# Abhipray/audio-codec

Hardware: AMD Instinct MI355X
Metric: audio channel-frames/s encode (48 kHz, 1024-line long blocks, 128 kb/s/ch) (higher is better)
Workload: dtype f64

## Files before the change

### audio-codec_amd/_lib.py

```python
import ctypes
import os

HERE = os.path.dirname(os.path.abspath(__file__))
LIB_PATH = os.environ.get("PACX_LIB") or os.path.join(HERE, "libpacx.so")

PACX_ABI_VERSION = 7
PCM_I16, PCM_F64 = 0, 1
FLAG_LAST, FLAG_CUR, FLAG_NEXT = 1, 2, 4
ST_SHORT, ST_ZERO_SUBBLOCK, ST_ALLOC_CAP, ST_VQ_UNDEFINED, ST_GUARD, ST_MALFORMED = 1, 2, 4, 8, 16, 32
ST_REF_RAISES = 64
ST_RATE_CAP = 128
RATE_STEP = 32
RATE_TARGET_GRID = 64
BAND_CAND = 16
E_ARG, E_UNSUPPORTED = -1, -2
REF_SCALAR_SBR_ERROR = "'numpy.int64' object does not support item assignment"
MAX_BANDS = 32
SUB = 8

c_double_p = ctypes.POINTER(ctypes.c_double)
c_int32_p = ctypes.POINTER(ctypes.c_int32)


class PacxSmrTables(ctypes.Structure):
# ... 58 lines not shown
class PacxPcm(ctypes.Structure):
    _fields_ = [
        ("data", ctypes.c_void_p),
        ("dtype", ctypes.c_int32),
        ("n_channels", ctypes.c_int32),
        ("n_frames", ctypes.c_int64),
        ("frame_stride", ctypes.c_int64),
        ("channel_stride", ctypes.c_int64),
        ("sample_stride", ctypes.c_int64),
    ]


_P = ctypes.c_void_p
SIGNATURES = {
    "pacx_abi_version": (ctypes.c_int, []),
    "pacx_create": (ctypes.c_int, [ctypes.POINTER(PacxConfig), ctypes.POINTER(_P)]),
    "pacx_destroy": (None, [_P]),
    "pacx_last_error": (ctypes.c_char_p, [_P]),
    "pacx_band_stride": (ctypes.c_int, [_P]),
    "pacx_payload_stride": (ctypes.c_int, [_P]),
    "pacx_reserve": (ctypes.c_int, [_P, ctypes.c_int64]),
    "pacx_tables_exact": (ctypes.c_int, [_P]),
    "pacx_default_bands": (ctypes.c_int, [ctypes.c_int, ctypes.c_int, c_int32_p, c_int32_p]),
    "pacx_mdct_batch": (ctypes.c_int, [_P, ctypes.POINTER(PacxPcm), _P, ctypes.c_int, _P, _P, _P]),
    "pacx_smr_batch": (ctypes.c_int, [_P, ctypes.POINTER(PacxPcm), _P, ctypes.c_int, _P, _P, _P, _P]),
    "pacx_bitalloc_batch": (ctypes.c_int, [_P, ctypes.c_int64, ctypes.c_int, _P, ctypes.c_int, _P, _P, _P, _P]),
    "pacx_quantize_batch": (ctypes.c_int, [_P, ctypes.c_int64, _P, _P, _P, ctypes.c_int, _P, _P, _P]),
    "pacx_encode_batch": (ctypes.c_int, [_P, ctypes.POINTER(PacxPcm), _P, _P, _P, _P, _P, _P, _P]),
    "pacx_encode_pack_batch": (ctypes.c_int, [_P, ctypes.POINTER(PacxPcm), _P, _P, _P, _P, _P, _P, _P, _P, _P]),
    "pacx_encode_vq_batch": (ctypes.c_int, [_P, ctypes.POINTER(PacxPcm), _P, _P, _P, _P, _P, _P, _P, _P,
                                            ctypes.c_int32, _P]),
    "pacx_pack_batch": (ctypes.c_int, [_P, ctypes.c_int64, ctypes.c_int, _P, _P, _P, _P, _P, _P, _P, _P, _P]),
    "pacx_gather_body": (ctypes.c_int, [_P, ctypes.c_int64, _P, _P, _P, ctypes.c_int64, _P, _P]),
    "pacx_window_batch": (ctypes.c_int, [_P, ctypes.c_int, ctypes.c_int64, _P, _P, _P]),
    "pacx_window_table_batch": (ctypes.c_int, [_P, _P, ctypes.c_int, ctypes.c_int64, _P, _P, _P]),
    "pacx_quantize_uniform": (ctypes.c_int, [_P, ctypes.c_int64, _P, ctypes.c_int, _P, _P]),
    "pacx_scale_factor": (ctypes.c_int, [_P, ctypes.c_int64, _P, ctypes.c_int, ctypes.c_int, _P, _P]),
    "pacx_mantissa": (ctypes.c_int, [_P, ctypes.c_int64, _P, ctypes.c_int, ctypes.c_int, ctypes.c_int, _P, _P]),
    "pacx_dequantize_uniform": (ctypes.c_int, [_P, ctypes.c_int64, _P, ctypes.c_int, _P, _P]),
    "pacx_dequantize": (ctypes.c_int, [_P, ctypes.c_int64, _P, ctypes.c_int, ctypes.c_int, ctypes.c_int, _P, _P]),
    "pacx_mantissa_fp": (ctypes.c_int, [_P, ctypes.c_int64, _P, ctypes.c_int, ctypes.c_int, ctypes.c_int, _P, _P]),
    "pacx_dequantize_fp": (ctypes.c_int, [_P, ctypes.c_int64, _P, ctypes.c_int, ctypes.c_int, ctypes.c_int, _P, _P]),
    "pacx_imdct_batch": (ctypes.c_int, [_P, ctypes.c_int64, ctypes.c_int, _P, _P, _P]),
    "pacx_mdct_direct_batch": (ctypes.c_int, [_P, ctypes.c_int64, ctypes.c_int, ctypes.c_int, ctypes.c_int, _P, _P, _P]),
    "pacx_transient_detect_f64": (ctypes.c_int, [_P, ctypes.c_int64, ctypes.c_int, ctypes.c_int, _P, ctypes.c_double, _P, _P]),
    "pacx_unpack_batch": (ctypes.c_int, [_P, ctypes.c_int64, _P, ctypes.c_int, _P, _P, _P, _P, _P, _P, _P, _P, _P]),
    "pacx_set_side_fork": (ctypes.c_int, [_P, ctypes.c_int]),
    "pacx_smr_generic_batch": (ctypes.c_int, [_P, ctypes.c_int64, ctypes.c_int, _P, _P, ctypes.POINTER(PacxSmrTables), _P, _P,
                                              _P, _P]),
    "pacx_decode_batch": (ctypes.c_int, [_P, ctypes.c_int64, ctypes.c_int, _P, _P, _P, _P, _P, _P, _P, _P]),
    "pacx_decode_sbr_batch": (ctypes.c_int, [_P, ctypes.c_int64, ctypes.c_int, _P, _P, _P, _P, _P, ctypes.c_int, _P, _P,
                                             _P, _P, _P]),
    "pacx_decode_vq_batch": (ctypes.c_int, [_P, ctypes.c_int64, ctypes.c_int, _P, ctypes.c_int, _P, _P, _P, _P, _P,
                                            _P, _P, _P, _P, _P]),
    "pacx_transient_flags": (ctypes.c_int, [_P, ctypes.POINTER(PacxPcm), _P, _P, _P]),
    "pacx_bitalloc_generic": (ctypes.c_int, [_P, ctypes.c_int64, ctypes.c_int, _P, _P, ctypes.c_int, _P, _P, _P]),
    "pacx_index_body": (ctypes.c_int, [_P, _P, ctypes.c_int64, ctypes.c_int, ctypes.c_int, ctypes.c_int64, _P, _P, _P, _P]),
    "pacx_overlap_add_pcm": (ctypes.c_int, [_P, ctypes.c_int64, ctypes.c_int, _P, _P, ctypes.c_int, _P, _P]),
    "pacx_nmr_batch": (ctypes.c_int, [_P, ctypes.POINTER(PacxPcm), _P, _P, _P, _P, _P, _P, _P, _P]),
    "pacx_nmr_summary": (ctypes.c_int, [_P, ctypes.c_int64, ctypes.c_int, _P, _P, _P, _P]),
    "pacx_encode_pack_nmr_batch": (ctypes.c_int, [_P, ctypes.POINTER(PacxPcm), _P, ctypes.c_double, ctypes.c_double,
                                                  _P, _P, _P, _P, _P, _P, _P, _P, _P]),
    "pacx_encode_pack_budget_batch": (ctypes.c_int, [_P, ctypes.POINTER(PacxPcm), _P, _P, _P, _P, _P, _P, _P, _P, _P,
                                                     _P]),
    "pacx_rate_curve_layout": (ctypes.c_int, [_P, ctypes.c_double, c_int32_p, c_int32_p]),
    "pacx_rate_curve_batch": (ctypes.c_int, [_P, ctypes.POINTER(PacxPcm), _P, ctypes.c_double, ctypes.c_int32, _P, _P, _P,
# ... 73 lines not shown
```

### audio-codec_amd/csrc/k_misc.hip

```cpp
#include "pacx_launch.h"

__global__ void k_window(const double *__restrict__ win, long long n_rows, int len,
                         const double *__restrict__ x, double *__restrict__ y)
{
    const long long i = (long long)blockIdx.x * blockDim.x + threadIdx.x;
    if (i < n_rows * len)
        y[i] = win[i % len] * x[i];
}

__global__ void k_quant_elem(int op, long long n, const double *__restrict__ x, int scale, int a, int b,
                             int64_t *__restrict__ out)
{
    const long long i = (long long)blockIdx.x * blockDim.x + threadIdx.x;
    if (i >= n)
        return;
    const double v = x[i];
    if (op == 0) {
        const int64_t mag = pacx_quant_mag(fabs(v), a);
        out[i] = (v < 0.0 ? ((int64_t)1 << (a - 1)) : 0) + mag;
    } else if (op == 1) {
        out[i] = pacx_scale_factor(fabs(v), a, b);
    } else if (op == 2) {
        out[i] = pacx_mantissa(v, scale, a, b);
    } else {
// ... 299 lines not shown
    if (lane == 63) {
        ws[wv] = ss;
        wl[wv] = sl;
    }
    __syncthreads();
    int at_s = ss - ns, at_l = sl - nl, all_s = 0, all_l = 0;
#pragma unroll
    for (int w = 0; w < NW; ++w) {
        at_s += w < wv ? ws[w] : 0;
        at_l += w < wv ? wl[w] : 0;
        all_s += ws[w];
        all_l += wl[w];
    }
    for (int j = 0; j < per; ++j) {
        if (!((valid >> j) & 1ull))
            break;
        const long long f = f0 + j;
        if ((shorts >> j) & 1ull) {
            for (int c = 0; c < n_ch; ++c)
                list_short[at_s * n_ch + c] = (int32_t)(f * n_ch + c);
            ++at_s;
        } else {
            for (int c = 0; c < n_ch; ++c)
                list_long[at_l * n_ch + c] = (int32_t)(f * n_ch + c);
            ++at_l;
        }
    }
    if (tid == 0) {
        counts[0] = all_l * n_ch;
        counts[1] = all_s * n_ch;
    }
}

void pacx_k::pacx_launch_frame_lists(const uint8_t *flags, long long n_frames, int n_ch, int32_t *list_long,
                             int32_t *list_short, int32_t *counts, hipStream_t st)
{
    if (n_frames <= 0)
        return;
    if (n_frames <= LISTS_SMALL_MAX) {
        hipLaunchKernelGGL(k_frame_lists_small, dim3(1), dim3(LISTS_SMALL_THREADS), 0, st, flags, n_frames, n_ch, list_long,
                           list_short, counts);
        return;
    }
    (void)hipMemsetAsync(counts, 0, 2 * sizeof(int32_t), st);
    hipLaunchKernelGGL(k_frame_lists, dim3((unsigned)((n_frames + 255) / 256)), dim3(256), 0, st, flags, n_frames,
                       n_ch, list_long, list_short, counts);
}

void pacx_k::pacx_launch_transient_f64(long long n_blocks, int n_ch, int n, const double *blocks, double thresh, uint8_t *out,
                               hipStream_t st)
{
    if (n_blocks > 0)
        hipLaunchKernelGGL(k_transient_f64, dim3((unsigned)n_blocks), dim3(64), 0, st, n_blocks, n_ch, n, blocks, thresh,
                           out);
}

void pacx_k::pacx_launch_transient(const PacxPcmView &in, long long n_hops, int hop, uint8_t *transient,
                           uint8_t *flags, hipStream_t st)
{
    if (n_hops > 0)
        hipLaunchKernelGGL(k_transient, dim3((unsigned)n_hops), dim3(64), 0, st, in, n_hops, hop, transient);
    if (flags)
        hipLaunchKernelGGL(k_stream_flags, dim3((unsigned)((n_hops + 2 + 255) / 256)), dim3(256), 0, st,
                           transient, n_hops, flags);
}

// ... 40 lines not shown
```

### audio-codec_amd/csrc/k_quant.hip

```cpp
#include "pacx_launch.h"
#include "wave_fft.h"
#include "quant_dev.h"

__global__ __launch_bounds__(64) void k_bitalloc(PacxTables T, const uint8_t *__restrict__ flags, int n_ch,
                                                long long n_cf, int short_blocks, int mixed, int skip_long,
                                                const double *__restrict__ smr,
                                                int32_t *__restrict__ bit_alloc,
                                                uint32_t *__restrict__ status)
{
    __shared__ double cp[2][32];
    const int lane = threadIdx.x, half = lane >> 5, l = lane & 31;
    const bool dense = !short_blocks && !(mixed && flags);
    const long long unit = (long long)blockIdx.x * 2 + half;
    const long long cf = dense ? unit : unit / PACX_SUB;
    const int sb = dense ? 0 : (int)(unit % PACX_SUB);
    bool alive = cf < n_cf;
    const unsigned fl = (alive && flags) ? flags[cf / n_ch] : 0u;
    const bool is_short = mixed ? ((fl & 2u) != 0) : (short_blocks != 0);
    if (!is_short && (sb != 0 || skip_long == 1))
        alive = false;
    if (is_short && skip_long == 2)
        alive = false;
    const int nb = is_short ? T.nb_short : T.nb_long;
    const int32_t *__restrict__ n_lines = is_short ? T.band_lines_short
// ... 592 lines not shown
            if (lane >= off)
                inc += t;
        }
        if (i < n_chunks)
            chunk_sum[i] = run + inc - v;
        run += __shfl(inc, 63, 64);
    }
    if (total && lane == 0)
        *total = run;
}

__global__ __launch_bounds__(256) void k_scan_offsets(const int32_t *__restrict__ n_bytes, long long n,
                                                     const long long *__restrict__ chunk_off,
                                                     long long *__restrict__ offs)
{
    __shared__ long long buf[256];
    const int t = threadIdx.x;
    const long long i = (long long)blockIdx.x * SCAN_CHUNK + t;
    const long long v = (i < n) ? rec_len(n_bytes[i]) : 0;
    buf[t] = v;
    __syncthreads();
    for (int off = 1; off < 256; off <<= 1) {
        const long long add = (t >= off) ? buf[t - off] : 0;
        __syncthreads();
        buf[t] += add;
        __syncthreads();
    }
    if (i < n)
        offs[i] = chunk_off[blockIdx.x] + buf[t] - v;
}

#define SCAN_SMALL_MAX 32768

__device__ __forceinline__ void copy_record(int nb, long long off, const uint8_t *__restrict__ src,
                                            uint8_t *__restrict__ body, long long capacity, int lane)
{
    if (nb <= 0 || off + nb + 4 > capacity)
        return;
    if (lane < 4)
        body[off + lane] = (uint8_t)((unsigned)nb >> (8 * lane));
    uint8_t *dst = body + off + 4;
    const int head = (int)((4 - ((uintptr_t)dst & 3)) & 3);
    if (lane < head && lane < nb)
        dst[lane] = src[lane];
    const int n_words = (nb - head) > 0 ? (nb - head) >> 2 : 0;
    for (int w = lane; w < n_words; w += 64) {
        const uint8_t *s = src + head + 4 * w;
        const unsigned v = (unsigned)s[0] | ((unsigned)s[1] << 8) | ((unsigned)s[2] << 16) | ((unsigned)s[3] << 24);
        *(unsigned *)(dst + head + 4 * w) = v;
    }
    const int done = head + 4 * n_words;
    if (done + lane < nb && lane < 4)
        dst[done + lane] = src[done + lane];
}

__global__ __launch_bounds__(64) void k_copy_body(const int32_t *__restrict__ n_bytes, long long n,
                                                 const long long *__restrict__ offs,
                                                 const uint8_t *__restrict__ payload, int payload_stride,
                                                 uint8_t *__restrict__ body, long long capacity)
{
    const long long i = blockIdx.x;
    if (i >= n)
        return;
    copy_record(n_bytes[i], offs[i], payload + i * (long long)payload_stride, body, capacity, threadIdx.x);
}

#define GATHER_REC 8
__global__ __launch_bounds__(256) void k_gather_small(const int32_t *__restrict__ n_bytes, long long n,
                                                     const uint8_t *__restrict__ payload, int payload_stride,
                                                     uint8_t *__restrict__ body, long long capacity,
                                                     long long *__restrict__ total)
{
    __shared__ int part[4];
    __shared__ int offs_s[GATHER_REC + 1];
    __shared__ int len_s[GATHER_REC];
    const int t = threadIdx.x, lane = t & 63, wv = t >> 6;
    const long long first = (long long)blockIdx.x * GATHER_REC;
    int acc = 0;
    const int4 *__restrict__ nb4 = (const int4 *)n_bytes;
    const int n4 = (int)(first >> 2);
#pragma unroll 8
    for (int j = t; j < n4; j += 256) {
        const int4 v = nb4[j];
        acc += (int)(rec_len(v.x) + rec_len(v.y) + rec_len(v.z) + rec_len(v.w));
    }
#pragma unroll
    for (int off = 32; off > 0; off >>= 1)
        acc += __shfl_xor(acc, off, 64);
    if (lane == 0)
        part[wv] = acc;
    __syncthreads();
    if (wv == 0) {
        const int base = part[0] + part[1] + part[2] + part[3];
        const int nb = (lane < GATHER_REC && first + lane < n) ? n_bytes[first + lane] : 0;
        const int len = (int)rec_len(nb);
        int incl = len;
#pragma unroll
        for (int off = 1; off < GATHER_REC; off <<= 1) {
            const int v = __shfl_up(incl, off, 64);
            if (lane >= off)
                incl += v;
        }
        if (lane < GATHER_REC) {
            offs_s[lane] = base + incl - len;
            len_s[lane] = nb;
        }
        if (lane == GATHER_REC - 1) {
            offs_s[GATHER_REC] = base + incl;
            if (total && first + GATHER_REC >= n)
                *total = (long long)(base + incl);
        }
    }
    __syncthreads();
    for (int r = wv; r < GATHER_REC && first + r < n; r += 4)
        copy_record(len_s[r], (long long)offs_s[r], payload + (first + r) * (long long)payload_stride, body,
                    capacity, lane);
}

void pacx_k::pacx_launch_bitalloc(const PacxTables &T, const uint8_t *flags, int n_ch, long long n_cf,
                          int short_blocks, int mixed, int skip_long, const double *smr, int32_t *bit_alloc,
                          uint32_t *status, hipStream_t st)
{
    if (n_cf <= 0)
        return;
    const bool dense = !short_blocks && !(mixed && flags);
    if (dense && skip_long == 1)
        return;
    const long long units = dense ? n_cf : n_cf * PACX_SUB;
    hipLaunchKernelGGL(k_bitalloc, dim3((unsigned)((units + 1) / 2)), dim3(64), 0, st, T, flags, n_ch,
                       n_cf, short_blocks, mixed, skip_long, smr, bit_alloc, status);
}

void pacx_k::pacx_launch_quantize(const PacxTables &T, const uint8_t *flags, int n_ch, long long n_cf,
                          int short_blocks, int mixed, const double *lines, const int32_t *overall,
                          int overall_stride, const int32_t *bit_alloc, int32_t *scale_factor,
                          int32_t *mantissa, hipStream_t st)
{
    if (n_cf <= 0)
        return;
    if (!short_blocks || mixed)
        hipLaunchKernelGGL((k_quantize<PACX_M_LONG>), dim3((unsigned)n_cf), dim3(64), 0, st, T, flags, n_ch,
                           n_cf, mixed, lines, overall, overall_stride, bit_alloc, scale_factor, mantissa);
    if (short_blocks || mixed)
        hipLaunchKernelGGL((k_quantize<PACX_M_SHORT>), dim3((unsigned)(n_cf * PACX_SUB)), dim3(64), 0, st, T,
                           flags, n_ch, n_cf * PACX_SUB, mixed, lines, overall, overall_stride, bit_alloc,
                           scale_factor, mantissa);
}

void pacx_k::pacx_launch_pack(const PacxTables &T, const uint8_t *flags, int n_ch, long long n_cf,
// ... 14 lines not shown
                      hipStream_t st)
{
    if (n_cf <= 0)
        return;
    const int mixed = flags ? 1 : 0;
    if (skip_long != 1)
        hipLaunchKernelGGL(k_tail_long, dim3((unsigned)(mixed ? n_cf : (n_cf + 1) / 2)), dim3(64), 0, st, T, flags,
                           n_ch, n_cf, mixed, smr, lines, overall, bit_alloc, scale_factor, mantissa, status, payload,
                           payload_stride, n_bytes);
    if (skip_long == 2)
        return;
    if (mixed && list_short && T.nb_short <= 8) {
        hipLaunchKernelGGL(k_tail_short, dim3((unsigned)n_cf), dim3(256), 0, st, T, flags, n_ch, list_short,
                           count_short, smr, lines, overall, bit_alloc, scale_factor, mantissa, status, payload,
                           payload_stride, n_bytes);
    } else if (mixed) {
        const long long units = n_cf * PACX_SUB;
        hipLaunchKernelGGL(k_bitalloc, dim3((unsigned)((units + 1) / 2)), dim3(64), 0, st, T, flags, n_ch, n_cf,
                           0, 1, 1, smr, bit_alloc, status);
        hipLaunchKernelGGL((k_quantize<PACX_M_SHORT>), dim3((unsigned)units), dim3(64), 0, st, T, flags, n_ch,
                           units, 1, lines, overall, PACX_SUB, bit_alloc, scale_factor, mantissa);
        if (payload)
            hipLaunchKernelGGL(k_pack, dim3((unsigned)n_cf), dim3(64), 0, st, T, flags, n_ch, n_cf, overall,
                               scale_factor, bit_alloc, mantissa, status, payload, payload_stride, n_bytes, 1);
    }
}

void pacx_k::pacx_launch_gather(long long n_cf, const uint8_t *payload, int payload_stride,
                        const int32_t *n_bytes, long long *chunk_buf, long long *offs_buf, uint8_t *body,
                        long long capacity, long long *total, hipStream_t st)
{
    if (n_cf <= 0)
        return;
    if (n_cf <= SCAN_SMALL_MAX) {
        hipLaunchKernelGGL(k_gather_small, dim3((unsigned)((n_cf + GATHER_REC - 1) / GATHER_REC)), dim3(256), 0, st,
                           n_bytes, n_cf, payload, payload_stride, body, capacity, total);
        return;
    }
    const long long n_chunks = (n_cf + SCAN_CHUNK - 1) / SCAN_CHUNK;
    hipLaunchKernelGGL(k_scan_partial, dim3((unsigned)n_chunks), dim3(256), 0, st, n_bytes, n_cf, chunk_buf);
    hipLaunchKernelGGL(k_scan_chunks, dim3(1), dim3(64), 0, st, chunk_buf, n_chunks, total);
    hipLaunchKernelGGL(k_scan_offsets, dim3((unsigned)n_chunks), dim3(256), 0, st, n_bytes, n_cf, chunk_buf,
                       offs_buf);
    hipLaunchKernelGGL(k_copy_body, dim3((unsigned)n_cf), dim3(64), 0, st, n_bytes, n_cf, offs_buf, payload,
                       payload_stride, body, capacity);
}
```

### audio-codec_amd/csrc/pacx_api.hip

```cpp
#include <hip/hip_runtime.h>

#include <math.h>
#include <stdio.h>
#include <stdlib.h>
#include <string.h>

#include <cmath>
#include <string>
#include <vector>

#include "../../include/pacx.h"
#include "body_index.h"
#include "pacx_launch.h"
#include "pvq_dev.h"
#include "pacx_vq_tables.h"
#include "pacx_tables_gen.h"

using namespace pacx_k;

struct PacxOverrides {
    int split_short;
    int fuse_tail;
    int fuse_front;
    int vq_fuse_alloc;
    int vq_frame;
    int vq_bfs;
    int vq_dec_frame;
};

#define PACX_FUSE_FRONT_DEFAULT 1

static int env_override(const char *name, int lo, int hi)
{
    const char *e = getenv(name);
    if (!e || !*e)
        return -1;
    char *end;
    const long v = strtol(e, &end, 10);
    return (*end || v < lo || v > hi) ? -1 : (int)v;
}

static PacxOverrides read_overrides(void)
{
    PacxOverrides o;
    o.split_short = env_override("PACX_SPLIT_SHORT", 0, 0);
    o.fuse_tail = env_override("PACX_FUSE_TAIL", 0, 1);
    o.fuse_front = env_override("PACX_FUSE_FRONT", 0, 1);
    o.vq_fuse_alloc = env_override("PACX_VQ_FUSE_ALLOC", 0, 1);
    o.vq_frame = env_override("PACX_VQ_FRAME", 0, 0);
    o.vq_bfs = env_override("PACX_VQ_BFS", 0, 1 << 20);
    o.vq_dec_frame = env_override("PACX_VQ_DEC_FRAME", 0, 0);
    return o;
}

struct pacx_handle {
    int device;
    int n_cu;
    PacxOverrides force;
    PacxTables T;
    std::vector<void *> owned;
    long long ws_cf;
    double *ws_lines;
    double *ws_smr;
    PacxPeak *ws_peaks;
    int32_t *ws_npeaks;
    int32_t *ws_nkept;
    int32_t *ws_overall;
    long long *ws_chunks;
    long long *ws_offs;
    int32_t *ws_lists;
    long long ws_blocks_cf;
    double *ws_blocks;
    int fork_side;
    hipStream_t side_stream;
    hipEvent_t ev_fork, ev_join;
    hipStream_t short_stream;
    hipStream_t spare_stream;
    hipEvent_t ev_short_done, ev_lists;
    std::vector<char> vq_view;
    std::vector<char> vqdec_view;
    int tables_exact;
    long long ws_mant_cf;
    int32_t *ws_mant;
    long long ws_dec_cf;
    double *ws_dec_lines;
    uint8_t *ws_dec_sbr;
    uint32_t *ws_dec_status;
    double *ws_sbr_mean;
    long long ws_vq_cf;
    unsigned *ws_unit_words;
// ... 212 lines not shown
    h->seg_host_n = 0;
    h->seg_host = nullptr;
    h->ev_seg = nullptr;
    h->ws_lines = nullptr; h->ws_smr = nullptr; h->ws_peaks = nullptr; h->ws_npeaks = nullptr;
    h->ws_overall = nullptr; h->ws_chunks = nullptr; h->ws_offs = nullptr; h->ws_nkept = nullptr;
    h->ws_lists = nullptr;
    h->tables_exact = 1;
    memset(&h->T, 0, sizeof(h->T));
    int rc = PACX_OK;
#define TRY(x) do { rc = (x); if (rc) { g_create_err = h->err; pacx_destroy(h); return rc; } } while (0)
    {
        hipError_t e = hipSetDevice(cfg->device);
        if (e != hipSuccess) {
            g_create_err = std::string("hipSetDevice: ") + hipGetErrorString(e);
            delete h;
            return PACX_E_HIP;
        }
    }
    if (hipStreamCreateWithFlags(&h->side_stream, hipStreamNonBlocking) != hipSuccess ||
        hipEventCreateWithFlags(&h->ev_fork, hipEventDisableTiming) != hipSuccess ||
        hipEventCreateWithFlags(&h->ev_join, hipEventDisableTiming) != hipSuccess ||
        hipStreamCreateWithFlags(&h->short_stream, hipStreamNonBlocking) != hipSuccess ||
        hipStreamCreateWithFlags(&h->spare_stream, hipStreamNonBlocking) != hipSuccess ||
        hipEventCreateWithFlags(&h->ev_short_done, hipEventDisableTiming) != hipSuccess ||
        hipEventCreateWithFlags(&h->ev_lists, hipEventDisableTiming) != hipSuccess) {
        g_create_err = "pacx_create: could not create the side stream / events";
        pacx_destroy(h);
        return PACX_E_HIP;
    }
    {
        hipDeviceProp_t prop;
        h->n_cu = (hipGetDeviceProperties(&prop, cfg->device) == hipSuccess && prop.multiProcessorCount > 0)
                      ? prop.multiProcessorCount : 256;
    }
    PacxTables &T = h->T;
    const int NL = PACX_N_LONG, NS = PACX_N_SHORT, ML = PACX_M_LONG, MS = PACX_M_SHORT;
    const double sr = cfg->sample_rate;

    std::vector<double> wl(4 * NL), ws(NS), hl(NL), hs(NS);
    if (cfg->win_long) {
        memcpy(wl.data(), cfg->win_long, sizeof(double) * 4 * NL);
    } else {
        const std::vector<double> sl = gen_table(PACX_GEN_SINE_LONG, NL), ss = gen_table(PACX_GEN_SINE_SHORT, NS);
        const int pad = NL / 4 - NS / 4;
        for (int i = 0; i < NL; ++i) {
            wl[i] = sl[i];
            double st;
            if (i < NL / 2) st = sl[i];
            else if (i < NL / 2 + pad) st = 1.0;
            else if (i < NL / 2 + pad + NS / 2) st = ss[NS / 2 + (i - NL / 2 - pad)];
            else st = 0.0;
            wl[NL + i] = st;
            double ssw;
            if (i < pad) ssw = 0.0;
            else if (i < pad + NS / 2) ssw = ss[i - pad];
            else if (i < pad + NS / 2 + 2 * pad) ssw = 1.0;
            else if (i < pad + NS + 2 * pad) ssw = ss[NS / 2 + (i - pad - NS / 2 - 2 * pad)];
            else ssw = 0.0;
            wl[3 * NL + i] = ssw;
        }
        for (int i = 0; i < NL; ++i)
            wl[2 * NL + i] = wl[NL + (NL - 1 - i)];
    }
    if (cfg->win_short) memcpy(ws.data(), cfg->win_short, sizeof(double) * NS);
    else ws = gen_table(PACX_GEN_SINE_SHORT, NS);
    if (cfg->hann_long) memcpy(hl.data(), cfg->hann_long, sizeof(double) * NL);
// ... 790 lines not shown
        return PACX_E_ARG;
    if (n_cf == 0)
        return PACX_OK;
    if (n_cf < 0 || n_channels < 1 || !overall_scale || !scale_factor || !bit_alloc || !mantissa || !payload ||
        !n_bytes)
        return fail(h, PACX_E_ARG, "pacx_pack_batch: bad argument");
    HIP_TRY(h, hipSetDevice(h->device));
    pacx_launch_pack(h->T, frame_flags, n_channels, n_cf, overall_scale, scale_factor, bit_alloc, mantissa,
                     status, payload, PACX_PAYLOAD_STRIDE, n_bytes, (hipStream_t)stream);
    return post_launch(h, "pacx_pack_batch");
}

extern "C" int pacx_gather_body(pacx_handle *h, int64_t n_cf, const uint8_t *payload, const int32_t *n_bytes,
                                uint8_t *body, int64_t body_capacity, int64_t *total_bytes, void *stream)
{
    if (!h)
        return PACX_E_ARG;
    if (n_cf == 0) {
        if (total_bytes)
            HIP_TRY(h, hipMemsetAsync(total_bytes, 0, sizeof(int64_t), (hipStream_t)stream));
        return PACX_OK;
    }
    if (n_cf < 0 || !payload || !n_bytes || !body || body_capacity < 0)
        return fail(h, PACX_E_ARG, "pacx_gather_body: bad argument");
    HIP_TRY(h, hipSetDevice(h->device));
    int rc = pacx_reserve(h, n_cf);
    if (rc)
        return rc;
    pacx_launch_gather(n_cf, payload, PACX_PAYLOAD_STRIDE, n_bytes, h->ws_chunks, h->ws_offs, body, body_capacity,
                       (long long *)total_bytes, (hipStream_t)stream);
    return post_launch(h, "pacx_gather_body");
}

extern "C" int pacx_window_batch(pacx_handle *h, int window, int64_t n_rows, const double *x, double *y,
                                 void *stream)
{
    if (!h)
        return PACX_E_ARG;
    if (n_rows < 0 || !x || !y)
        return fail(h, PACX_E_ARG, "pacx_window_batch: bad argument");
    const double *w;
    int len;
    switch (window) {
    case PACX_WIN_SINE: case PACX_WIN_START: case PACX_WIN_STOP: case PACX_WIN_STARTSTOP:
        w = h->T.win_long + window * PACX_N_LONG; len = PACX_N_LONG; break;
    case PACX_WIN_SINE_SHORT: w = h->T.win_short; len = PACX_N_SHORT; break;
    case PACX_WIN_HANN: w = h->T.hann_long; len = PACX_N_LONG; break;
    case PACX_WIN_HANN_SHORT: w = h->T.hann_short; len = PACX_N_SHORT; break;
    case PACX_WIN_KBD: w = h->T.kbd_long; len = PACX_N_LONG; break;
    case PACX_WIN_KBD_SHORT: w = h->T.kbd_short; len = PACX_N_SHORT; break;
    default: return fail(h, PACX_E_ARG, "pacx_window_batch: unknown window");
    }
    HIP_TRY(h, hipSetDevice(h->device));
    pacx_launch_window(w, n_rows, len, x, y, (hipStream_t)stream);
    return post_launch(h, "pacx_window_batch");
}

extern "C" int pacx_window_table_batch(pacx_handle *h, const double *table, int len, int64_t n_rows,
                                       const double *x, double *y, void *stream)
{
    if (!h)
        return PACX_E_ARG;
    if (n_rows < 0 || len < 1 || !table || !x || !y)
        return fail(h, PACX_E_ARG, "pacx_window_table_batch: bad argument");
    HIP_TRY(h, hipSetDevice(h->device));
    pacx_launch_window(table, n_rows, len, x, y, (hipStream_t)stream);
// ... 709 lines not shown
```

### audio-codec_amd/csrc/pacx_launch.h

```cpp
#ifndef PACX_LAUNCH_H
#define PACX_LAUNCH_H

#include "../../include/pacx.h"
#include "pacx_dev.h"

struct PvqTables;

namespace pacx_k {

void pacx_launch_mdct(const PacxTables &T, const PacxPcmView &in, int dtype, int fast,
                      const uint8_t *flags, long long n_cf, int short_blocks, int mixed, int prewin,
                      double *lines, int32_t *scale_out, int scale_stride, uint32_t *status,
                      hipStream_t st);
void pacx_launch_mdct_v2(const PacxTables &T, const PacxPcmView &in, const uint8_t *flags, long long n_cf,
                         int skip_cur, double *lines, int32_t *scale_out, int scale_stride,
                         uint32_t *status_init, int n_cu, const int32_t *cf_list, const int32_t *cf_count,
                         hipStream_t st);
void pacx_launch_mdct_x2(const PacxTables &T, const PacxPcmView &in, long long n_cf, double *lines,
                         int32_t *scale_out, int scale_stride, uint32_t *status_init, int n_cu, hipStream_t st);

void pacx_launch_side(const PacxTables &T, const PacxPcmView &in, int dtype, int fast,
                      const uint8_t *flags, long long n_cf, int short_blocks, int mixed,
                      PacxPeak *peaks, int32_t *n_peaks, int32_t *n_kept, double *sbr_mean,
                      int32_t *sbr_overall, hipStream_t st);
// ... 2 lines not shown
                            int32_t *n_kept, hipStream_t st);
void pacx_launch_mask(const PacxTables &T, const uint8_t *flags, int n_ch, long long n_cf,
                      int short_blocks, int mixed, const PacxPeak *peaks, const int32_t *n_peaks,
                      const double *lines, double *smr, double *thr_out, int n_cu,
                      const int32_t *list_long, const int32_t *list_short, const int32_t *counts,
                      const MaskTail *tail, hipStream_t st);
size_t pacx_smr_generic_lds(int n);
void pacx_launch_smr_generic(long long n_blocks, int n, int nb, const double *data, const double *lines,
                             const double *hann, const double *tw_cos, const double *tw_sin, double norm, double fstep,
                             const double *bark, const double *quiet, const int32_t *band_lower,
                             const int32_t *band_count, double *smr, double *thr_out, int32_t *n_peaks_out,
                             hipStream_t st);

void pacx_launch_bitalloc(const PacxTables &T, const uint8_t *flags, int n_ch, long long n_cf,
                          int short_blocks, int mixed, int skip_long, const double *smr, int32_t *bit_alloc,
                          uint32_t *status, hipStream_t st);
void pacx_launch_quantize(const PacxTables &T, const uint8_t *flags, int n_ch, long long n_cf,
                          int short_blocks, int mixed, const double *lines, const int32_t *overall,
                          int overall_stride, const int32_t *bit_alloc, int32_t *scale_factor,
                          int32_t *mantissa, hipStream_t st);
void pacx_launch_pack(const PacxTables &T, const uint8_t *flags, int n_ch, long long n_cf,
                      const int32_t *overall, const int32_t *scale_factor, const int32_t *bit_alloc,
                      const int32_t *mantissa, const uint32_t *status, uint8_t *payload,
                      int payload_stride, int32_t *n_bytes, hipStream_t st);
void pacx_launch_tail(const PacxTables &T, const uint8_t *flags, int n_ch, long long n_cf, const double *smr,
                      const double *lines, const int32_t *overall, int32_t *bit_alloc, int32_t *scale_factor,
                      int32_t *mantissa, uint32_t *status, uint8_t *payload, int payload_stride,
                      int32_t *n_bytes, const int32_t *list_short, const int32_t *count_short, int skip_long,
                      hipStream_t st);
void pacx_launch_gather(long long n_cf, const uint8_t *payload, int payload_stride,
                        const int32_t *n_bytes, long long *chunk_buf, long long *offs_buf, uint8_t *body,
                        long long capacity, long long *total, hipStream_t st);

void pacx_launch_frame_lists(const uint8_t *flags, long long n_frames, int n_ch, int32_t *list_long,
                             int32_t *list_short, int32_t *counts, hipStream_t st);
void pacx_launch_window(const double *win, long long n_rows, int len, const double *x, double *y,
                        hipStream_t st);
void pacx_launch_quant_elem(int op, long long n, const double *x, int scale, int a, int b, int64_t *out,
                            hipStream_t st);
void pacx_launch_dequant_elem(int op, long long n, const int64_t *codes, int scale, int a, int b, double *out,
                              hipStream_t st);
void pacx_launch_mdct_direct(long long n_rows, int a, int b, int inverse, const double *x, double *y, hipStream_t st);
void pacx_launch_bitalloc_generic(long long n, int nb, const int32_t *n_lines, const double *budget,
                                  int max_mant, const double *smr, int32_t *bits, hipStream_t st);
void pacx_launch_transient_f64(long long n_blocks, int n_ch, int n, const double *blocks, double thresh, uint8_t *out,
                               hipStream_t st);
void pacx_launch_transient(const PacxPcmView &in, long long n_hops, int hop, uint8_t *transient,
                           uint8_t *flags, hipStream_t st);

void pacx_launch_imdct_plain(const PacxTables &T, long long n_rows, int short_blocks, const double *lines,
                             double *blocks, hipStream_t st);
void pacx_launch_sbr_scalar_lines(const PacxTables &T, long long n_cf, const uint8_t *cf_flags,
                                  const int32_t *scale_factor, const int32_t *bit_alloc, const int32_t *mantissa,
                                  double *lines, uint8_t *sbr_flag, int routing, hipStream_t st);
void pacx_launch_unpack(const PacxTables &T, long long n_cf, const uint8_t *payload, int payload_stride,
                        const long long *offsets, const int32_t *n_bytes, uint8_t *flags_out, int32_t *overall,
                        int32_t *scale_factor, int32_t *bit_alloc, int32_t *mantissa, uint32_t *status,
                        hipStream_t st);
void pacx_launch_decode(const PacxTables &T, long long n_blocks, int n_ch, const uint8_t *cf_flags,
                        const int32_t *overall, const int32_t *scale_factor, const int32_t *bit_alloc,
                        const int32_t *mantissa, const double *lines_in, double *blocks, int16_t *pcm,
                        hipStream_t st);
void pacx_launch_ola_tail(long long n_blocks, int n_ch, const double *blocks, double *tail, int flush, int16_t *pcm,
                          hipStream_t st);

size_t pacx_index_ws_bytes(long long n_body, PacxIndexWs *ws);
// ... 91 lines not shown
```

### audio-codec_amd/engine.py

```python
import ctypes

import numpy as np
import torch

from . import _lib, tables
from .psychoac import ScaleFactorBands, AssignMDCTLinesFromFreqLimits

N_LONG, N_SHORT = 1024, 128


def _ptr(t):
    return ctypes.c_void_p(t.data_ptr()) if t is not None else None


class PcmView:

    def __init__(self, tensor, n_channels, n_frames, frame_stride, channel_stride,
                 sample_stride=1):
        if tensor.dtype == torch.int16:
            dt = _lib.PCM_I16
        elif tensor.dtype == torch.float64:
            dt = _lib.PCM_F64
        else:
            raise TypeError("PCM must be int16 codes or float64 signed fractions")
        if not tensor.is_cuda:
            raise ValueError("PCM tensor must live on the GPU")
        self.tensor = tensor
        self.n_channels, self.n_frames = int(n_channels), int(n_frames)
        if self.n_frames > 0 and self.n_channels > 0:
            last = (self.n_frames - 1) * max(int(frame_stride), 0) + (self.n_channels - 1) * max(int(channel_stride), 0) \
                + (2 * N_LONG - 1) * max(int(sample_stride), 0)
            have = tensor.untyped_storage().nbytes() // tensor.element_size() - tensor.storage_offset()
            if last >= have:
# ... 621 lines not shown
        return out

    def transient_detect(self, blocks, thresh=4.5):
        blocks = blocks.contiguous()
        n, n_ch, ln = blocks.shape
        out = self._empty((n,), torch.uint8)
        self._call("pacx_transient_detect_f64", ctypes.c_int64(n), int(n_ch), int(ln), _ptr(blocks),
                   ctypes.c_double(float(thresh)), _ptr(out), self._stream())
        return out

    def bit_alloc_generic(self, budget, max_mant_bits, n_lines, smr):
        smr = smr.contiguous()
        n, nb = smr.shape
        nl = torch.as_tensor(np.asarray(n_lines, dtype=np.int32), device=self.device)
        bits = self._empty((n, nb), torch.int32)
        self._call("pacx_bitalloc_generic", ctypes.c_int64(n), int(nb), _ptr(nl), _ptr(budget.contiguous()),
                   int(max_mant_bits), _ptr(smr), _ptr(bits), self._stream())
        return bits


class EncoderPool:

    def __init__(self, n, *args, **kwargs):
        self.encs = [Encoder(*args, **kwargs) for _ in range(max(1, int(n)))]
        dev = self.encs[0].device
        self.streams = [torch.cuda.Stream(device=dev) for _ in self.encs]
        self.done = [torch.cuda.Event() for _ in self.encs]
        self._turn = 0
        self._gate = self._gate_stream = None
        self._used = [False] * len(self.encs)
        if len(self.encs) > 1:
            for e in self.encs:
                e.set_side_fork(True)

    def __len__(self):
        return len(self.encs)

    def next(self):
        k = self._turn
        self._turn = (k + 1) % len(self.encs)
        return k

    def slot(self, k):
        pool = self

        class _Slot:
            def __enter__(self_inner):
                self_inner.ctx = torch.cuda.stream(pool.streams[k])
                self_inner.ctx.__enter__()
                return pool.encs[k]

            def __exit__(self_inner, *exc):
                pool.done[k].record(pool.streams[k])
                pool._used[k] = True
                return self_inner.ctx.__exit__(*exc)
        return _Slot()

    def align(self, delay_us=None):
        if len(self.encs) < 2:
            return
        if delay_us is None:
            delay_us = float(os.environ.get("PACX_POOL_GATE_US", "100"))
        if delay_us <= 0 or not hasattr(torch.cuda, "_sleep"):
            return
        dev = self.encs[0].device
        if self._gate is None:
            self._gate_stream = torch.cuda.Stream(device=dev)
            self._gate = torch.cuda.Event()
            t0, t1 = torch.cuda.Event(enable_timing=True), torch.cuda.Event(enable_timing=True)
            with torch.cuda.stream(self._gate_stream):
                torch.cuda._sleep(100_000)
                t0.record()
                torch.cuda._sleep(2_000_000)
                t1.record()
            t1.synchronize()
            self._cycles_per_us = 2_000_000 / max(t0.elapsed_time(t1) * 1e3, 1.0)
        with torch.cuda.stream(self._gate_stream):
            for k in range(len(self.encs)):
                if self._used[k]:
                    self._gate_stream.wait_event(self.done[k])
            torch.cuda._sleep(int(delay_us * self._cycles_per_us))
            self._gate.record(self._gate_stream)
        for s in self.streams:
            s.wait_event(self._gate)

    def wait(self, k, stream=None):
        (stream or torch.cuda.current_stream(self.encs[0].device)).wait_event(self.done[k])

    def synchronize(self):
        for s in self.streams:
            s.synchronize()

    def close(self):
        for e in self.encs:
            e.close()
```

### include/pacx.h

```cpp
#ifndef PACX_H
#define PACX_H

#include <stdint.h>

#ifdef __cplusplus
extern "C" {
#endif

#define PACX_ABI_VERSION 7

#define PACX_OK            0
#define PACX_E_ARG        -1
#define PACX_E_UNSUPPORTED -2
#define PACX_E_HIP        -3
#define PACX_E_NOMEM      -4

#define PACX_PCM_I16 0
#define PACX_PCM_F64 1

#define PACX_FLAG_LAST 1u
#define PACX_FLAG_CUR  2u
#define PACX_FLAG_NEXT 4u

#define PACX_WIN_SINE 0
// ... 104 lines not shown
                        void *stream);

int pacx_quantize_batch(pacx_handle *h, int64_t n_cf, const double *lines,
                        const int32_t *overall_scale, const int32_t *bit_alloc,
                        int short_blocks, int32_t *scale_factor, int32_t *mantissa,
                        void *stream);


int pacx_encode_batch(pacx_handle *h, const pacx_pcm *in, const uint8_t *frame_flags,
                      int32_t *overall_scale, int32_t *scale_factor,
                      int32_t *bit_alloc, int32_t *mantissa, uint32_t *status,
                      void *stream);

int pacx_encode_pack_batch(pacx_handle *h, const pacx_pcm *in, const uint8_t *frame_flags,
                           int32_t *overall_scale, int32_t *scale_factor, int32_t *bit_alloc,
                           int32_t *mantissa, uint32_t *status, uint8_t *payload, int32_t *n_bytes,
                           void *stream);

int pacx_encode_vq_batch(pacx_handle *h, const pacx_pcm *in, const uint8_t *frame_flags,
                         int32_t *overall_scale, int32_t *bit_alloc, uint8_t *payload,
                         int32_t *n_bytes, uint32_t *status, pacx_vq_entry *entries,
                         int32_t *entry_count, int32_t entries_per_band, void *stream);

int pacx_pack_batch(pacx_handle *h, int64_t n_cf, int n_channels,
                    const uint8_t *frame_flags, const int32_t *overall_scale,
                    const int32_t *scale_factor, const int32_t *bit_alloc,
                    const int32_t *mantissa, const uint32_t *status,
                    uint8_t *payload, int32_t *n_bytes, void *stream);

int pacx_gather_body(pacx_handle *h, int64_t n_cf, const uint8_t *payload,
                     const int32_t *n_bytes, uint8_t *body, int64_t body_capacity,
                     int64_t *total_bytes, void *stream);


int pacx_window_batch(pacx_handle *h, int window, int64_t n_rows, const double *x, double *y,
                      void *stream);
int pacx_window_table_batch(pacx_handle *h, const double *table, int len, int64_t n_rows,
                            const double *x, double *y, void *stream);
int pacx_quantize_uniform(pacx_handle *h, int64_t n, const double *x, int n_bits, int64_t *codes,
                          void *stream);
int pacx_scale_factor(pacx_handle *h, int64_t n, const double *x, int n_scale_bits, int n_mant_bits,
                      int64_t *scale, void *stream);
int pacx_mantissa(pacx_handle *h, int64_t n, const double *x, int scale, int n_scale_bits,
                  int n_mant_bits, int64_t *mantissa, void *stream);
int pacx_dequantize_uniform(pacx_handle *h, int64_t n, const int64_t *codes, int n_bits, double *x,
                            void *stream);
int pacx_dequantize(pacx_handle *h, int64_t n, const int64_t *mantissa, int scale, int n_scale_bits,
                    int n_mant_bits, double *x, void *stream);
int pacx_mantissa_fp(pacx_handle *h, int64_t n, const double *x, int scale, int n_scale_bits,
                     int n_mant_bits, int64_t *mantissa, void *stream);
int pacx_dequantize_fp(pacx_handle *h, int64_t n, const int64_t *mantissa, int scale, int n_scale_bits,
                       int n_mant_bits, double *x, void *stream);
int pacx_imdct_batch(pacx_handle *h, int64_t n_rows, int mode, const double *lines, double *blocks,
                     void *stream);
int pacx_mdct_direct_batch(pacx_handle *h, int64_t n_rows, int a, int b, int inverse, const double *x,
                           double *y, void *stream);
int pacx_bitalloc_generic(pacx_handle *h, int64_t n, int n_bands, const int32_t *band_lines,
                          const double *budget, int max_mant_bits, const double *smr,
                          int32_t *bit_alloc, void *stream);

int pacx_transient_flags(pacx_handle *h, const pacx_pcm *hops, uint8_t *transient,
                         uint8_t *frame_flags, void *stream);

int pacx_transient_detect_f64(pacx_handle *h, int64_t n_blocks, int n_channels, int n_samples,
                              const double *blocks, double thresh, uint8_t *result, void *stream);

// ... 126 lines not shown
```

Measured before the change: 52.43 million.

## Use aligned word copies in body gather and replace torch sleep gate with native delay kernel

The body gather and copy kernels get an aligned variant. It reads 32-bit words from the payload slot and realigns them with a funnel shift instead of assembling each word from four byte loads. It is selected at launch when the payload pointer and stride are 4-byte aligned. The prefix-sum loop in the small gather is manually two-way unrolled, and per-record lengths and offsets are made wave-uniform. Separately, the pool gate no longer uses torch's _sleep with a calibration pass; a new wall-clock-based delay kernel runs on stream 0, which avoids an extra stream and the calibration sync.

```diff
diff --git a/audio-codec_amd/_lib.py b/audio-codec_amd/_lib.py
--- a/audio-codec_amd/_lib.py
+++ b/audio-codec_amd/_lib.py
@@ -114,6 +114,7 @@
                                             ctypes.c_int32, _P]),
     "pacx_pack_batch": (ctypes.c_int, [_P, ctypes.c_int64, ctypes.c_int, _P, _P, _P, _P, _P, _P, _P, _P, _P]),
     "pacx_gather_body": (ctypes.c_int, [_P, ctypes.c_int64, _P, _P, _P, ctypes.c_int64, _P, _P]),
+    "pacx_stream_delay": (ctypes.c_int, [_P, ctypes.c_double, _P]),
     "pacx_window_batch": (ctypes.c_int, [_P, ctypes.c_int, ctypes.c_int64, _P, _P, _P]),
     "pacx_window_table_batch": (ctypes.c_int, [_P, _P, ctypes.c_int, ctypes.c_int64, _P, _P, _P]),
     "pacx_quantize_uniform": (ctypes.c_int, [_P, ctypes.c_int64, _P, ctypes.c_int, _P, _P]),
diff --git a/audio-codec_amd/csrc/k_misc.hip b/audio-codec_amd/csrc/k_misc.hip
--- a/audio-codec_amd/csrc/k_misc.hip
+++ b/audio-codec_amd/csrc/k_misc.hip
@@ -355,6 +355,24 @@
     }
 }
 
+__global__ __launch_bounds__(64) void k_stream_delay(long long ticks)
+{
+    if (threadIdx.x != 0)
+        return;
+    const long long t0 = (long long)wall_clock64();
+    for (long long i = 0; i < ticks; ++i) {
+        if ((long long)wall_clock64() - t0 >= ticks)
+            break;
+        __builtin_amdgcn_s_sleep(8);
+    }
+}
+
+void pacx_k::pacx_launch_stream_delay(long long ticks, hipStream_t st)
+{
+    if (ticks > 0)
+        hipLaunchKernelGGL(k_stream_delay, dim3(1), dim3(64), 0, st, ticks);
+}
+
 void pacx_k::pacx_launch_frame_lists(const uint8_t *flags, long long n_frames, int n_ch, int32_t *list_long,
                              int32_t *list_short, int32_t *counts, hipStream_t st)
 {
diff --git a/audio-codec_amd/csrc/k_quant.hip b/audio-codec_amd/csrc/k_quant.hip
--- a/audio-codec_amd/csrc/k_quant.hip
+++ b/audio-codec_amd/csrc/k_quant.hip
@@ -648,7 +648,8 @@
 
 #define SCAN_SMALL_MAX 32768
 
-__device__ __forceinline__ void copy_record(int nb, long long off, const uint8_t *__restrict__ src,
+template <bool ALIGNED>
+__device__ __forceinline__ void copy_record(int nb, long long off, const uint8_t *__restrict__ src, int slot_words,
                                             uint8_t *__restrict__ body, long long capacity, int lane)
 {
     if (nb <= 0 || off + nb + 4 > capacity)
@@ -660,14 +661,37 @@
     if (lane < head && lane < nb)
         dst[lane] = src[lane];
     const int n_words = (nb - head) > 0 ? (nb - head) >> 2 : 0;
-    for (int w = lane; w < n_words; w += 64) {
-        const uint8_t *s = src + head + 4 * w;
-        const unsigned v = (unsigned)s[0] | ((unsigned)s[1] << 8) | ((unsigned)s[2] << 16) | ((unsigned)s[3] << 24);
-        *(unsigned *)(dst + head + 4 * w) = v;
+    if (ALIGNED) {
+        const unsigned *__restrict__ s32 = (const unsigned *)src;
+        unsigned *__restrict__ d32 = (unsigned *)(dst + head);
+        const int last = slot_words - 1, sh = 8 * head;
+#pragma clang loop unroll(disable) vectorize(disable) interleave(disable)
+        for (int w = lane; w < n_words; w += 64) {
+            const unsigned lo = s32[w], hi = s32[w + 1 < last ? w + 1 : last];
+            d32[w] = (unsigned)((((unsigned long long)hi << 32) | lo) >> sh);
+        }
+    } else {
+        for (int w = lane; w < n_words; w += 64) {
+            const uint8_t *s = src + head + 4 * w;
+            const unsigned v = (unsigned)s[0] | ((unsigned)s[1] << 8) | ((unsigned)s[2] << 16) | ((unsigned)s[3] << 24);
+            *(unsigned *)(dst + head + 4 * w) = v;
+        }
     }
     const int done = head + 4 * n_words;
     if (done + lane < nb && lane < 4)
         dst[done + lane] = src[done + lane];
+}
+
+template <bool ALIGNED>
+__device__ __forceinline__ void copy_body(const int32_t *__restrict__ n_bytes, long long n,
+                                          const long long *__restrict__ offs, const uint8_t *__restrict__ payload,
+                                          int payload_stride, uint8_t *__restrict__ body, long long capacity)
+{
+    const long long i = blockIdx.x;
+    if (i >= n)
+        return;
+    copy_record<ALIGNED>(n_bytes[i], offs[i], payload + i * (long long)payload_stride, payload_stride >> 2, body,
+                         capacity, threadIdx.x);
 }
 
 __global__ __launch_bounds__(64) void k_copy_body(const int32_t *__restrict__ n_bytes, long long n,
@@ -675,28 +699,40 @@
                                                  const uint8_t *__restrict__ payload, int payload_stride,
                                                  uint8_t *__restrict__ body, long long capacity)
 {
-    const long long i = blockIdx.x;
-    if (i >= n)
-        return;
-    copy_record(n_bytes[i], offs[i], payload + i * (long long)payload_stride, body, capacity, threadIdx.x);
+    copy_body<true>(n_bytes, n, offs, payload, payload_stride, body, capacity);
+}
+
+__global__ __launch_bounds__(64) void k_copy_body_bytes(const int32_t *__restrict__ n_bytes, long long n,
+                                                       const long long *__restrict__ offs,
+                                                       const uint8_t *__restrict__ payload, int payload_stride,
+                                                       uint8_t *__restrict__ body, long long capacity)
+{
+    copy_body<false>(n_bytes, n, offs, payload, payload_stride, body, capacity);
 }
 
 #define GATHER_REC 8
-__global__ __launch_bounds__(256) void k_gather_small(const int32_t *__restrict__ n_bytes, long long n,
-                                                     const uint8_t *__restrict__ payload, int payload_stride,
-                                                     uint8_t *__restrict__ body, long long capacity,
-                                                     long long *__restrict__ total)
+template <bool ALIGNED>
+__device__ __forceinline__ void gather_small(const int32_t *__restrict__ n_bytes, long long n,
+                                             const uint8_t *__restrict__ payload, int payload_stride,
+                                             uint8_t *__restrict__ body, long long capacity,
+                                             long long *__restrict__ total)
 {
     __shared__ int part[4];
-    __shared__ int offs_s[GATHER_REC + 1];
+    __shared__ int offs_s[GATHER_REC];
     __shared__ int len_s[GATHER_REC];
-    const int t = threadIdx.x, lane = t & 63, wv = t >> 6;
+    const int t = threadIdx.x, lane = t & 63, wv = __builtin_amdgcn_readfirstlane(t >> 6);
     const long long first = (long long)blockIdx.x * GATHER_REC;
     int acc = 0;
     const int4 *__restrict__ nb4 = (const int4 *)n_bytes;
-    const int n4 = (int)(first >> 2);
-#pragma unroll 8
-    for (int j = t; j < n4; j += 256) {
+    const unsigned n4 = (unsigned)(first >> 2);
+    unsigned j = t;
+#pragma clang loop unroll(disable) vectorize(disable) interleave(disable)
+    for (; j + 256 < n4; j += 512) {
+        const int4 v = nb4[j], u = nb4[j + 256];
+        acc += (int)(rec_len(v.x) + rec_len(v.y) + rec_len(v.z) + rec_len(v.w));
+        acc += (int)(rec_len(u.x) + rec_len(u.y) + rec_len(u.z) + rec_len(u.w));
+    }
+    if (j < n4) {
         const int4 v = nb4[j];
         acc += (int)(rec_len(v.x) + rec_len(v.y) + rec_len(v.z) + rec_len(v.w));
     }
@@ -721,16 +757,31 @@
             offs_s[lane] = base + incl - len;
             len_s[lane] = nb;
         }
-        if (lane == GATHER_REC - 1) {
-            offs_s[GATHER_REC] = base + incl;
-            if (total && first + GATHER_REC >= n)
-                *total = (long long)(base + incl);
-        }
-    }
-    __syncthreads();
-    for (int r = wv; r < GATHER_REC && first + r < n; r += 4)
-        copy_record(len_s[r], (long long)offs_s[r], payload + (first + r) * (long long)payload_stride, body,
-                    capacity, lane);
+        if (lane == GATHER_REC - 1 && total && first + GATHER_REC >= n)
+            *total = (long long)(base + incl);
+    }
+    __syncthreads();
+    for (int r = wv; r < GATHER_REC && first + r < n; r += 4) {
+        const int nb = __builtin_amdgcn_readfirstlane(len_s[r]), off = __builtin_amdgcn_readfirstlane(offs_s[r]);
+        copy_record<ALIGNED>(nb, (long long)off, payload + (first + r) * (long long)payload_stride, payload_stride >> 2,
+                             body, capacity, lane);
+    }
+}
+
+__global__ __launch_bounds__(256) void k_gather_small(const int32_t *__restrict__ n_bytes, long long n,
+                                                     const uint8_t *__restrict__ payload, int payload_stride,
+                                                     uint8_t *__restrict__ body, long long capacity,
+                                                     long long *__restrict__ total)
+{
+    gather_small<true>(n_bytes, n, payload, payload_stride, body, capacity, total);
+}
+
+__global__ __launch_bounds__(256) void k_gather_small_bytes(const int32_t *__restrict__ n_bytes, long long n,
+                                                           const uint8_t *__restrict__ payload, int payload_stride,
+                                                           uint8_t *__restrict__ body, long long capacity,
+                                                           long long *__restrict__ total)
+{
+    gather_small<false>(n_bytes, n, payload, payload_stride, body, capacity, total);
 }
 
 void pacx_k::pacx_launch_bitalloc(const PacxTables &T, const uint8_t *flags, int n_ch, long long n_cf,
@@ -811,8 +862,10 @@
 {
     if (n_cf <= 0)
         return;
+    const bool aligned = ((uintptr_t)payload & 3) == 0 && (payload_stride & 3) == 0;
     if (n_cf <= SCAN_SMALL_MAX) {
-        hipLaunchKernelGGL(k_gather_small, dim3((unsigned)((n_cf + GATHER_REC - 1) / GATHER_REC)), dim3(256), 0, st,
+        hipLaunchKernelGGL(aligned ? k_gather_small : k_gather_small_bytes,
+                           dim3((unsigned)((n_cf + GATHER_REC - 1) / GATHER_REC)), dim3(256), 0, st,
                            n_bytes, n_cf, payload, payload_stride, body, capacity, total);
         return;
     }
@@ -821,6 +874,6 @@
     hipLaunchKernelGGL(k_scan_chunks, dim3(1), dim3(64), 0, st, chunk_buf, n_chunks, total);
     hipLaunchKernelGGL(k_scan_offsets, dim3((unsigned)n_chunks), dim3(256), 0, st, n_bytes, n_cf, chunk_buf,
                        offs_buf);
-    hipLaunchKernelGGL(k_copy_body, dim3((unsigned)n_cf), dim3(64), 0, st, n_bytes, n_cf, offs_buf, payload,
-                       payload_stride, body, capacity);
-}
+    hipLaunchKernelGGL(aligned ? k_copy_body : k_copy_body_bytes, dim3((unsigned)n_cf), dim3(64), 0, st, n_bytes, n_cf,
+                       offs_buf, payload, payload_stride, body, capacity);
+}
diff --git a/audio-codec_amd/csrc/pacx_api.hip b/audio-codec_amd/csrc/pacx_api.hip
--- a/audio-codec_amd/csrc/pacx_api.hip
+++ b/audio-codec_amd/csrc/pacx_api.hip
@@ -56,6 +56,7 @@
 struct pacx_handle {
     int device;
     int n_cu;
+    int wall_khz;
     PacxOverrides force;
     PacxTables T;
     std::vector<void *> owned;
@@ -334,6 +335,9 @@
         hipDeviceProp_t prop;
         h->n_cu = (hipGetDeviceProperties(&prop, cfg->device) == hipSuccess && prop.multiProcessorCount > 0)
                       ? prop.multiProcessorCount : 256;
+        int khz = 0;
+        h->wall_khz = (hipDeviceGetAttribute(&khz, hipDeviceAttributeWallClockRate, cfg->device) == hipSuccess && khz > 0)
+                          ? khz : 100000;
     }
     PacxTables &T = h->T;
     const int NL = PACX_N_LONG, NS = PACX_N_SHORT, ML = PACX_M_LONG, MS = PACX_M_SHORT;
@@ -1190,6 +1194,20 @@
     return post_launch(h, "pacx_gather_body");
 }
 
+extern "C" int pacx_stream_delay(pacx_handle *h, double delay_us, void *stream)
+{
+    if (!h)
+        return PACX_E_ARG;
+    if (!(delay_us <= 10000.0))
+        return fail(h, PACX_E_ARG, "pacx_stream_delay: delay_us must be at most 10000");
+    if (delay_us <= 0.0)
+        return PACX_OK;
+    HIP_TRY(h, hipSetDevice(h->device));
+    const long long ticks = (long long)(delay_us * (double)h->wall_khz * 1e-3 + 0.5);
+    pacx_launch_stream_delay(ticks, (hipStream_t)stream);
+    return post_launch(h, "pacx_stream_delay");
+}
+
 extern "C" int pacx_window_batch(pacx_handle *h, int window, int64_t n_rows, const double *x, double *y,
                                  void *stream)
 {
diff --git a/audio-codec_amd/csrc/pacx_launch.h b/audio-codec_amd/csrc/pacx_launch.h
--- a/audio-codec_amd/csrc/pacx_launch.h
+++ b/audio-codec_amd/csrc/pacx_launch.h
@@ -58,6 +58,7 @@
                         const int32_t *n_bytes, long long *chunk_buf, long long *offs_buf, uint8_t *body,
                         long long capacity, long long *total, hipStream_t st);
 
+void pacx_launch_stream_delay(long long ticks, hipStream_t st);
 void pacx_launch_frame_lists(const uint8_t *flags, long long n_frames, int n_ch, int32_t *list_long,
                              int32_t *list_short, int32_t *counts, hipStream_t st);
 void pacx_launch_window(const double *win, long long n_rows, int len, const double *x, double *y,
diff --git a/audio-codec_amd/engine.py b/audio-codec_amd/engine.py
--- a/audio-codec_amd/engine.py
+++ b/audio-codec_amd/engine.py
@@ -1,4 +1,5 @@
 import ctypes
+import os
 
 import numpy as np
 import torch
@@ -686,6 +687,13 @@
         if len(self.encs) > 1:
             for e in self.encs:
                 e.set_side_fork(True)
+            self._gate_stream = self.streams[0]
+            self._gate = torch.cuda.Event()
+            self._delay(1.0)
+
+    def _delay(self, delay_us):
+        self.encs[0]._call("pacx_stream_delay", ctypes.c_double(float(delay_us)),
+                           ctypes.c_void_p(self._gate_stream.cuda_stream))
 
     def __len__(self):
         return len(self.encs)
@@ -715,28 +723,16 @@
             return
         if delay_us is None:
             delay_us = float(os.environ.get("PACX_POOL_GATE_US", "100"))
-        if delay_us <= 0 or not hasattr(torch.cuda, "_sleep"):
+        if delay_us <= 0:
             return
-        dev = self.encs[0].device
-        if self._gate is None:
-            self._gate_stream = torch.cuda.Stream(device=dev)
-            self._gate = torch.cuda.Event()
-            t0, t1 = torch.cuda.Event(enable_timing=True), torch.cuda.Event(enable_timing=True)
-            with torch.cuda.stream(self._gate_stream):
-                torch.cuda._sleep(100_000)
-                t0.record()
-                torch.cuda._sleep(2_000_000)
-                t1.record()
-            t1.synchronize()
-            self._cycles_per_us = 2_000_000 / max(t0.elapsed_time(t1) * 1e3, 1.0)
-        with torch.cuda.stream(self._gate_stream):
-            for k in range(len(self.encs)):
-                if self._used[k]:
-                    self._gate_stream.wait_event(self.done[k])
-            torch.cuda._sleep(int(delay_us * self._cycles_per_us))
-            self._gate.record(self._gate_stream)
+        for k in range(len(self.encs)):
+            if self._used[k] and k != 0:
+                self._gate_stream.wait_event(self.done[k])
+        self._delay(delay_us)
+        self._gate.record(self._gate_stream)
         for s in self.streams:
-            s.wait_event(self._gate)
+            if s is not self._gate_stream:
+                s.wait_event(self._gate)
 
     def wait(self, k, stream=None):
         (stream or torch.cuda.current_stream(self.encs[0].device)).wait_event(self.done[k])
diff --git a/include/pacx.h b/include/pacx.h
--- a/include/pacx.h
+++ b/include/pacx.h
@@ -160,6 +160,8 @@
                      const int32_t *n_bytes, uint8_t *body, int64_t body_capacity,
                      int64_t *total_bytes, void *stream);
 
+int pacx_stream_delay(pacx_handle *h, double delay_us, void *stream);
+
 
 int pacx_window_batch(pacx_handle *h, int window, int64_t n_rows, const double *x, double *y,
                       void *stream);
```

Result: faster. 54.89 million, median of 6 (+4.7%).
